# redmod-team/SympGPR

Measured on AMD Instinct MI355X. Metric: Gram-build GB/s + Cholesky fp64 TFLOP/s at N=65536 d=2; |alpha-alpha_ref|/|alpha_ref|, higher is better.
Workload: dtype f64

## Files before the change

### sympgpr_amd/csrc/chol.hip

```cpp
#include <algorithm>
#include <cstdlib>
#include <mutex>
#include <vector>

#include "cholq.h"
#include "common.h"
#include "gemm_tile.h"
#include "leaf.h"

namespace sgpr {

namespace {

using namespace leaf;


__global__ __launch_bounds__(LT) void leaf_kernel(int nb, double *A, size_t lda, double *inv,
                                                  int *dinfo, int goff, int mode,
                                                  unsigned long long *stamps)
{
    __shared__ double s[LEAF_LDS];
    if (nb == LEAF) leaf_body(s, (int)LEAF, A, lda, inv, dinfo, goff, mode, stamps);
    else            leaf_body(s, nb, A, lda, inv, dinfo, goff, mode, stamps);
}
// ... 476 lines not shown
            idx[0] = F0 + cp * PW_MAX + g;
            return panel_wait_ge(a.flags, idx, 1, 3, a.dinfo, sh + 1, a.abort);
        };
        for (int c = 0; c + 1 < g; ++c) {
            double *X = tileptr(g, c);
            XTile x;
            CTile cd;
            if (!wait_helper(c)) return false;
            asm volatile("s_waitcnt vmcnt(0)" ::: "memory");
            __syncthreads();
            trsm_prefetch(X, a.lda, x);
            diag_prefetch(tileptr(g, g), a.lda, cd);
            idx[0] = E0 + c;
            if (!panel_wait(a.flags, idx, 1, a.dinfo, sh + 1, a.abort)) return false;
            trsm_solve(s, tileptr(c, c), a.inv + (size_t)c * LEAF * LEAF, a.lda, x);
            trsm_store(X, a.lda, x);
            panel_publish_wt(a.flags + F0 + g * PW_MAX + c);
            diag_update_global(s, x, cd, tileptr(g, g), a.lda);
            if (c == 0 && a.NH > 0) claim_tiles();
            int cnt = 0;
            for (int cc = c + 1; cc < g; ++cc)
                if (!((helped >> cc) & 1u)) idx[cnt++] = F0 + cc * PW_MAX + c;
            if (cnt && !panel_wait(a.flags, idx, cnt, a.dinfo, sh + 1, a.abort)) return false;
            for (int t = 1; t < g - c; ++t)
                if (!((helped >> (c + t)) & 1u))
                    panel_product(s, -1.0, X, a.lda, tileptr(c + t, c), a.lda, 1.0, tileptr(g, c + t), a.lda);
        }
        if (g > 0) {
            const int c = g - 1;
            double *X = tileptr(g, c);
            XTile x;
            CTile cd;
            if (!wait_helper(c)) return false;
            asm volatile("s_waitcnt vmcnt(0)" ::: "memory");
            __syncthreads();
            trsm_prefetch(X, a.lda, x);
            diag_prefetch(tileptr(g, g), a.lda, cd);
            idx[0] = E0 + c;
            if (dbg) a.dbg[16 * g + 2] = __builtin_amdgcn_s_memrealtime();
            if (!panel_wait(a.flags, idx, 1, a.dinfo, sh + 1, a.abort)) return false;
            if (dbg) a.dbg[16 * g + 0] = __builtin_amdgcn_s_memrealtime();
            trsm_solve(s, tileptr(c, c), a.inv + (size_t)c * LEAF * LEAF, a.lda, x, a.dbg ? a.dbg + 16 * g + 6 : nullptr);
            trsm_store(X, a.lda, x);
            if (dbg) a.dbg[16 * g + 1] = __builtin_amdgcn_s_memrealtime();
            diag_update_into_leaf(s, x, cd, a.dbg ? a.dbg + 16 * g + 8 : nullptr);
            if (tid == 0) __hip_atomic_store((gint *)(a.flags + F0 + g * PW_MAX + c), 1, __ATOMIC_RELAXED, __HIP_MEMORY_SCOPE_AGENT);
        }
        asm volatile("s_waitcnt vmcnt(0)" ::: "memory");
        __syncthreads();
        if (dbg) a.dbg[16 * g + 4] = __builtin_amdgcn_s_memrealtime();
        leaf_body(s, (int)LEAF, tileptr(g, g), a.lda,
                  a.inv + (size_t)g * LEAF * LEAF, a.dinfo, a.goff + g * LEAF, (int)LEAF_FACTOR, nullptr,
                  a.flags + E0 + g, g > 0, dbg ? a.dbg + 16 * g + 11 : nullptr);
        panel_publish(a.flags + 2 + g);
        if (a.abort && tid == 0)
            __hip_atomic_fetch_add((gint *)(a.abort + (cholq::Q_PROG - cholq::Q_ABORT)), 1, __ATOMIC_RELAXED, __HIP_MEMORY_SCOPE_AGENT);
        if (dbg) a.dbg[16 * g + 5] = __builtin_amdgcn_s_memrealtime();
        if (cen && tid == 0) cen[2] = __builtin_amdgcn_s_memrealtime();
        return true;
    }
    if (g < W + a.NH) {
        int h = g - W, cp = 1, gg = 2;
        while (h >= W - 1 - cp) { h -= W - 1 - cp; ++cp; }
        gg = cp + 1 + h;
        int *word = a.flags + F0 + cp * PW_MAX + gg;
        if (tid == 0) sh[1] = atomicCAS(word, 0, 1);
        __syncthreads();
        const int old = sh[1];
        __syncthreads();
        if (old != 0) return true;
        if (a.ver) {
            idx[0] = ((a.ver_i0 + (gg >> 1)) * a.ver_ld + a.ver_j0 + cp) * (int)cholq::VS;
            if (!panel_wait_ge(a.ver, idx, 1, a.ver_need, a.dinfo, sh + 1, a.abort)) return false;
        }
        for (int c = 0; c < cp; ++c) {
            idx[0] = F0 + gg * PW_MAX + c;
            idx[1] = F0 + cp * PW_MAX + c;
            if (!panel_wait(a.flags, idx, 2, a.dinfo, sh + 1, a.abort)) return false;
            panel_product(s, -1.0, tileptr(gg, c), a.lda, tileptr(cp, c), a.lda, 1.0, tileptr(gg, cp), a.lda);
        }
        panel_publish_val(word, 3);
        return true;
    }
    const int gb = g - a.NH;
    if (a.tiles) {
        const int nbel = R - W, ntiles = nbel * W;
        int *const counter = a.flags + 2 * PFLAG_STRIDE - 1;
        for (;;) {
            if (tid == 0) sh[1] = atomicAdd(counter, 1);
            __syncthreads();
            const int q = sh[1];
            __syncthreads();
            if (q >= ntiles) return true;
            const int cp = q / nbel, r = W + q % nbel;
            const int pword = PFLAG_STRIDE + (r - W);
            if (a.ver) {
                idx[0] = ((a.ver_i0 + (r >> 1)) * a.ver_ld + a.ver_j0 + cp) * (int)cholq::VS;
                if (!panel_wait_ge(a.ver, idx, 1, a.ver_need, a.dinfo, sh + 1, a.abort)) return false;
            }
            for (int c = 0; c < cp; ++c) {
                idx[0] = pword;
                if (!panel_wait_ge(a.flags, idx, 1, c + 1, a.dinfo, sh + 1, a.abort)) return false;
                idx[0] = F0 + cp * PW_MAX + c;
                if (!panel_wait(a.flags, idx, 1, a.dinfo, sh + 1, a.abort)) return false;
                panel_product(s, -1.0, tileptr(r, c), a.lda, tileptr(cp, c), a.lda, 1.0, tileptr(r, cp), a.lda);
            }
            {
                double *X = tileptr(r, cp);
                XTile x;
                asm volatile("s_waitcnt vmcnt(0)" ::: "memory");
                __syncthreads();
                trsm_prefetch(X, a.lda, x);
                idx[0] = E0 + cp;
                if (!panel_wait(a.flags, idx, 1, a.dinfo, sh + 1, a.abort)) return false;
                trsm_solve(s, tileptr(cp, cp), a.inv + (size_t)cp * LEAF * LEAF, a.lda, x);
                trsm_store(X, a.lda, x);
            }
            asm volatile("s_waitcnt vmcnt(0)" ::: "memory");
            __syncthreads();
            if (tid == 0) __hip_atomic_store((gint *)(a.flags + pword), cp + 1, __ATOMIC_RELAXED, __HIP_MEMORY_SCOPE_AGENT);
            if (cp == W - 1) {
                if (a.tver) panel_publish_val(a.tver + (size_t)(a.tver_r0 + r) * cholq::VS, a.tver_val);
                if (a.abort && tid == 0)
                    __hip_atomic_fetch_add((gint *)(a.abort + (cholq::Q_PROG - cholq::Q_ABORT)), 1, __ATOMIC_RELAXED, __HIP_MEMORY_SCOPE_AGENT);
            }
        }
    }
    const int nw = G - W;
    const int r_first = W + (gb - W), r_step = nw > 0 ? nw : R;
    if (a.ver) {
        const int vi = a.ver_i0 + (r_first >> 1);
        for (int c = 0; c < W; ++c) idx[c] = (vi * a.ver_ld + a.ver_j0 + c) * (int)cholq::VS;
        if (r_first < R && !panel_wait_ge(a.ver, idx, W, a.ver_need, a.dinfo, sh + 1, a.abort)) return false;
    }
    const bool below_early = a.below_early != 0;
    for (int c = 0; c < W; ++c) {
        bool have_inv = false, have_early = false, have_rows = false;
        for (int r = r_first; r < R; r += r_step) {
            double *X = tileptr(r, c);
            if (c == W - 1 || below_early) {
                XTile x;
                asm volatile("s_waitcnt vmcnt(0)" ::: "memory");
                __syncthreads();
                trsm_prefetch(X, a.lda, x);
                if (!have_early) {
                    idx[0] = E0 + c;
                    if (!panel_wait(a.flags, idx, 1, a.dinfo, sh + 1, a.abort)) return false;
                    have_early = true;
                }
                trsm_solve(s, tileptr(c, c), a.inv + (size_t)c * LEAF * LEAF, a.lda, x);
                trsm_store(X, a.lda, x);
                if (c == W - 1) continue;
            } else {
                if (!have_inv) {
                    idx[0] = 2 + c;
                    if (!panel_wait(a.flags, idx, 1, a.dinfo, sh + 1, a.abort)) return false;
                    have_inv = true;
                }
                panel_product(s, 1.0, X, a.lda, a.inv + (size_t)c * LEAF * LEAF, (size_t)LEAF, 0.0, X, a.lda);
            }
            for (int t = 1; t <= W - 1 - c; ++t) {
                if (t == 1 && !have_rows) {
                    int cnt = 0;
                    for (int cc = c + 1; cc < W; ++cc) idx[cnt++] = F0 + cc * PW_MAX + c;
                    if (cnt && !panel_wait(a.flags, idx, cnt, a.dinfo, sh + 1, a.abort)) return false;
                    have_rows = true;
                }
                panel_product(s, -1.0, X, a.lda, tileptr(c + t, c), a.lda, 1.0, tileptr(r, c + t), a.lda);
            }
        }
    }
    if (a.tver && r_first < R) panel_publish_val(a.tver + (size_t)(a.tver_r0 + r_first) * cholq::VS, a.tver_val);
    if (a.abort && tid == 0)
        __hip_atomic_fetch_add((gint *)(a.abort + (cholq::Q_PROG - cholq::Q_ABORT)), 1, __ATOMIC_RELAXED, __HIP_MEMORY_SCOPE_AGENT);
    if (cen && tid == 0) cen[2] = __builtin_amdgcn_s_memrealtime();
    return true;
}

__global__ __launch_bounds__(LT) void panel_kernel(const PanelArgs a)
{
    __shared__ double s[LEAF * ILD];
    __shared__ int sh[2];
    static_assert(2 * tile::BK * 2 * (LEAF + tile::PAD) <= LEAF_LDS && LEAF_LDS <= LEAF * ILD, "product staging and the leaf fit the buffer");
    const int tid = threadIdx.x;
    const int W = a.W, G = a.G;
    if (tid == 0) {
        int t = -1;
        if ((blockIdx.x & 7) == 0) {
            t = atomicAdd(a.flags, 1);
            if (t >= W) t = -1;
        }
        if (t < 0) t = W + atomicAdd(a.flags + 1, 1);
        sh[0] = t;
    }
    __syncthreads();
    const int g = sh[0];
    __syncthreads();
    if (g >= G + a.NH) return;
    (void)panel_strip(a, g, s, sh);
}

struct PanelSeq {
    double *A;
    size_t lda;
    int nblk;
    int nblk_all;
    const int *pstart;
    double *inv;
    int *dinfo;
    int goff;
    int *flags;
    const int *ver;
    int ver_ld;
    int *tver;
    int *abort;
    unsigned long long *census;
    int helpers, tiles;
};

__global__ __launch_bounds__(LT) void panel_seq_kernel(const PanelSeq q)
{
    __shared__ double s[LEAF * ILD];
    __shared__ int sh[2];
    const int g = blockIdx.x;
    for (int k = 0; k < q.nblk; ++k) {
        const int k0 = q.pstart[k], w = q.pstart[k + 1] - k0, wnext = k + 1 < q.nblk_all ? q.pstart[k + 2] - q.pstart[k + 1] : 0;
        PanelArgs a{};
        a.P = q.A + k0 + (size_t)k0 * q.lda; a.lda = q.lda;
        a.W = w / LEAF;
        a.R = a.G = (w + wnext) / LEAF;
        a.below_early = q.tiles;
        a.NH = (q.helpers && a.W > 2 && a.G + (a.W - 1) * (a.W - 2) / 2 <= (int)gridDim.x) ? (a.W - 1) * (a.W - 2) / 2 : 0;
        if (q.tiles && wnext > 0 && a.W >= 2 && (int)gridDim.x - a.W - a.NH >= 1) {
            a.tiles = 1;
            a.G = a.W + min((int)gridDim.x - a.W - a.NH, (a.R - a.W) * a.W);
        }
        a.inv = q.inv + (size_t)(k0 / LEAF) * LEAF * LEAF;
        a.dinfo = q.dinfo; a.goff = q.goff + k0;
        a.flags = q.flags + (size_t)(k0 / LEAF) * PFLAG_STRIDE;
        a.dbg = nullptr;
        a.ver = q.ver; a.ver_ld = q.ver_ld; a.ver_i0 = k0 / cholq::TM; a.ver_j0 = k0 / cholq::TN; a.ver_need = k0 / LEAF;
        a.tver = q.tver; a.tver_r0 = k0 / LEAF; a.tver_val = (k0 + w) / LEAF;
        a.abort = q.abort;
        a.census = (q.census && k < (int)cholq::TRACE_PANELS) ? q.census + 4 * cholq::TRACE_PANEL_WGS * (size_t)k : nullptr;
        if (g < a.G + a.NH && !panel_strip(a, g, s, sh)) return;
        asm volatile("s_waitcnt vmcnt(0)" ::: "memory");
        __syncthreads();
    }
}

struct PanelBatch {
    double *A;
    size_t stride_a, lda;
    double *inv;
    size_t stride_inv;
    int *flags;
    int *info;
    int *ticket;
    int W, nbatch;
    int R;
    int k0;
    int G;
};

__global__ __launch_bounds__(LT) void panel_batch_kernel(const PanelBatch q)
{
    __shared__ double s[LEAF * ILD];
    __shared__ int sh[2];
    if (threadIdx.x == 0) sh[0] = atomicAdd(q.ticket, 1);
    __syncthreads();
    const int t = sh[0];
    __syncthreads();
    const int p = t / q.G, g = t - p * q.G;
    if (p >= q.nbatch) return;
    PanelArgs a{};
    a.P = q.A + (size_t)p * q.stride_a + (size_t)q.k0 + (size_t)q.k0 * q.lda; a.lda = q.lda;
    a.W = q.W; a.R = q.R; a.G = q.G;
    a.inv = q.inv + (size_t)p * q.stride_inv + (size_t)(q.k0 / (int)LEAF) * LEAF * LEAF;
    a.dinfo = q.info + p; a.goff = q.k0;
    a.flags = q.flags + (size_t)p * PFLAG_STRIDE;
    a.below_early = 1;
    (void)panel_strip(a, g, s, sh);
}

inline int split(int n)
{
    int n1 = ((n / 2 + LEAF - 1) / LEAF) * LEAF;
    if (n1 >= n) n1 -= LEAF;
    return n1;
}

struct Ctx {
    double *inv;
    int *dinfo;
    hipStream_t st;
    int la_max = 0;
    int *flags = nullptr;
    void *qws = nullptr;
};

int potrf_lookahead(int n, double *A, size_t lda, const Ctx &c, int nb, int off0);
inline int la_block(int n) { return n <= 4096 ? 256 : (n <= 24576 ? 512 : (n <= 40960 ? 1024 : 2048)); }

int trsm_rec(int m, int n, const double *L, size_t ldl, double *B, size_t ldb, int off, const Ctx &c)
{
    if (n <= LEAF) {
        return gemm_nt(m, n, n, 1.0, B, ldb, c.inv + (size_t)(off / LEAF) * LEAF * LEAF, LEAF, 0.0,
                       B, ldb, 0, 0, c.st);
    }
    const int n1 = split(n), n2 = n - n1;
    int rc = trsm_rec(m, n1, L, ldl, B, ldb, off, c);
    if (rc) return rc;
    rc = gemm_nt(m, n2, n1, -1.0, B, ldb, L + n1, ldl, 1.0, B + (size_t)n1 * ldb, ldb, 0, 0, c.st);
    if (rc) return rc;
    return trsm_rec(m, n2, L + n1 + (size_t)n1 * ldl, ldl, B + (size_t)n1 * ldb, ldb, off + n1, c);
}

int trsm_rl_rec(int m, int n, const double *L, size_t ldl, double *B, size_t ldb, int off, const Ctx &c)
{
    if (n <= LEAF)
        return gemm_nn(m, n, n, 1.0, B, ldb, c.inv + (size_t)(off / LEAF) * LEAF * LEAF, LEAF, 0.0, B, ldb, c.st);
    const int n1 = split(n), n2 = n - n1;
    int rc = trsm_rl_rec(m, n2, L + n1 + (size_t)n1 * ldl, ldl, B + (size_t)n1 * ldb, ldb, off + n1, c);
    if (rc) return rc;
    rc = gemm_nn(m, n1, n2, -1.0, B + (size_t)n1 * ldb, ldb, L + n1, ldl, 1.0, B, ldb, c.st);
    if (rc) return rc;
    return trsm_rl_rec(m, n1, L, ldl, B, ldb, off, c);
}

int potrf_rec(int n, double *A, size_t lda, int off, const Ctx &c)
{
    if (n <= LEAF) {
        hipLaunchKernelGGL(leaf_kernel, dim3(1), dim3(LT), 0, c.st, n, A, lda,
                           c.inv + (size_t)(off / LEAF) * LEAF * LEAF, c.dinfo, off, (int)LEAF_FACTOR,
                           (unsigned long long *)nullptr);
        SGPR_CHECK_LAUNCH();
        return 0;
    }
    if (n > 4 * LEAF && n <= c.la_max) return potrf_lookahead(n, A, lda, c, 0, off);
    const int n1 = split(n), n2 = n - n1;
    double *A21 = A + n1, *A22 = A + n1 + (size_t)n1 * lda;
    int rc = potrf_rec(n1, A, lda, off, c);
    if (rc) return rc;
    rc = trsm_rec(n2, n1, A, lda, A21, lda, off, c);
    if (rc) return rc;
    rc = gemm_nt(n2, n2, n1, -1.0, A21, lda, A21, lda, 1.0, A22, lda, 1, 0, c.st);
    if (rc) return rc;
    return potrf_rec(n2, A22, lda, off + n1, c);
}

int trsv_n_rec(int n, const double *L, size_t ldl, double *b, int off, const Ctx &c)
{
    if (n <= LEAF) {
        hipLaunchKernelGGL(leaf_matvec_kernel, dim3(1), dim3(MV_T), 0, c.st, n,
                           c.inv + (size_t)(off / LEAF) * LEAF * LEAF, b, 0);
        SGPR_CHECK_LAUNCH();
        return 0;
    }
    if (n <= TRSV_BLOCK) {
        hipLaunchKernelGGL(trsv_block_kernel, dim3(1), dim3(MV_T), 0, c.st, n, L, ldl,
                           c.inv + (size_t)(off / LEAF) * LEAF * LEAF, b, 0);
        SGPR_CHECK_LAUNCH();
        return 0;
    }
    const int n1 = split(n), n2 = n - n1;
    int rc = trsv_n_rec(n1, L, ldl, b, off, c);
    if (rc) return rc;
    rc = gemv_n_sub(n2, n1, L + n1, ldl, b, b + n1, c.st);
    if (rc) return rc;
    return trsv_n_rec(n2, L + n1 + (size_t)n1 * ldl, ldl, b + n1, off + n1, c);
}

int trsv_t_rec(int n, const double *L, size_t ldl, double *b, int off, const Ctx &c)
{
    if (n <= LEAF) {
        hipLaunchKernelGGL(leaf_matvec_kernel, dim3(1), dim3(MV_T), 0, c.st, n,
                           c.inv + (size_t)(off / LEAF) * LEAF * LEAF, b, 1);
        SGPR_CHECK_LAUNCH();
        return 0;
    }
    if (n <= TRSV_BLOCK) {
        hipLaunchKernelGGL(trsv_block_kernel, dim3(1), dim3(MV_T), 0, c.st, n, L, ldl,
                           c.inv + (size_t)(off / LEAF) * LEAF * LEAF, b, 1);
        SGPR_CHECK_LAUNCH();
        return 0;
    }
    const int n1 = split(n), n2 = n - n1;
    int rc = trsv_t_rec(n2, L + n1 + (size_t)n1 * ldl, ldl, b + n1, off + n1, c);
    if (rc) return rc;
    rc = gemv_t_sub(n2, n1, L + n1, ldl, b + n1, b, c.st);
    if (rc) return rc;
    return trsv_t_rec(n1, L, ldl, b, off, c);
}

int leaves_invert_only(int n, double *L, size_t ldl, const Ctx &c)
{
    for (int off = 0; off < n; off += LEAF) {
        const int nb = n - off < LEAF ? n - off : LEAF;
        hipLaunchKernelGGL(leaf_kernel, dim3(1), dim3(LT), 0, c.st, nb, L + off + (size_t)off * ldl, ldl,
                           c.inv + (size_t)(off / LEAF) * LEAF * LEAF, c.dinfo, off,
                           (int)LEAF_INVERT_ONLY, (unsigned long long *)nullptr);
        SGPR_CHECK_LAUNCH();
    }
    return 0;
}

inline size_t inv_bytes(int n)
{
    return (size_t)((n + LEAF - 1) / LEAF) * LEAF * LEAF * sizeof(double);
}
inline size_t flag_bytes(int n)
{
    return (((size_t)((n + LEAF - 1) / LEAF) * PFLAG_STRIDE * sizeof(int)) + 255) / 256 * 256;
}


}

inline size_t pub_bytes(int n) { return ((size_t)2 * n * sizeof(double) + 255) / 256 * 256; }
size_t potrf_workspace(int n) { return n <= 0 ? 256 : inv_bytes(n) + flag_bytes(n) + pub_bytes(n) + cholq::ws_bytes(n) + 256; }

namespace {

struct EventPool {
    std::vector<hipEvent_t> ev;
    size_t top = 0;
};
thread_local EventPool t_event_pool[64];

struct EventSet {
    std::vector<hipEvent_t> ev;
    EventPool *pool = nullptr;
    size_t base = 0;
    int create(size_t count)
    {
        int dev = 0;
        SGPR_HIP(hipGetDevice(&dev));
        if (dev < 0 || dev >= 64) { set_error("potrf: device index out of range"); return SGPR_E_ARG; }
        pool = &t_event_pool[dev];
        base = pool->top;
        while (pool->ev.size() < base + count) {
            hipEvent_t e = nullptr;
            SGPR_HIP(hipEventCreateWithFlags(&e, hipEventDisableTiming));
            pool->ev.push_back(e);
        }
        pool->top = base + count;
        ev.assign(pool->ev.begin() + (long)base, pool->ev.begin() + (long)(base + count));
        return 0;
    }
    ~EventSet()
    {
        if (pool) pool->top = base;
    }
};
struct StreamJoin {
    hipStream_t side, caller;
    hipEvent_t ev;
    ~StreamJoin()
    {
        if (hipEventRecord(ev, side) != hipSuccess || hipStreamWaitEvent(caller, ev, 0) != hipSuccess)
            (void)hipStreamSynchronize(side);
        gemm_set_overlap(0);
    }
};

hipStream_t g_side[64] = {};
std::mutex g_side_mu;

void release_all_streams_at_exit();
void register_exit_release()
{
    static std::once_flag once;
    std::call_once(once, [] { (void)atexit(release_all_streams_at_exit); });
}

int side_stream(hipStream_t caller, hipStream_t *out, int *dev_out)
{
    hipStream_t *const side = g_side;
    int dev = -1;
    if (caller) {
        SGPR_HIP(hipStreamGetDevice(caller, &dev));
    } else {
        SGPR_HIP(hipGetDevice(&dev));
    }
    if (dev < 0 || dev >= 64) { set_error("potrf: device index out of range"); return SGPR_E_ARG; }
    std::lock_guard<std::mutex> lock(g_side_mu);
    if (!side[dev]) {
        int cur = -1, lo = 0, hi = 0;
        SGPR_HIP(hipGetDevice(&cur));
        if (cur != dev) SGPR_HIP(hipSetDevice(dev));
        hipError_t e = hipDeviceGetStreamPriorityRange(&lo, &hi);
        if (e == hipSuccess) e = hipStreamCreateWithPriority(&side[dev], hipStreamNonBlocking, hi);
        if (e == hipSuccess) register_exit_release();
        if (cur != dev) (void)hipSetDevice(cur);
        SGPR_HIP(e);
    }
    *out = side[dev];
    *dev_out = dev;
    return 0;
}

struct QueueDevice {
    std::mutex mu;
    hipEvent_t done = nullptr;
    int ncu = 0;
    hipStream_t workers[4] = {}, panels[4] = {};
    bool overlap_ok[4] = {};
    bool failed = false;
};
QueueDevice g_qdev[64];

__global__ void overlap_probe_kernel(int *w, int me)
{
    __hip_atomic_store((gint *)(w + me), 1, __ATOMIC_RELAXED, __HIP_MEMORY_SCOPE_AGENT);
    const unsigned long long t0 = __builtin_amdgcn_s_memrealtime();
    int seen = 0;
    while (!(seen = __hip_atomic_load((gint *)(w + 1 - me), __ATOMIC_RELAXED, __HIP_MEMORY_SCOPE_AGENT))) {
        __builtin_amdgcn_s_sleep(32);
        if (__builtin_amdgcn_s_memrealtime() - t0 > 5000000ull) break;
    }
    w[2 + me] = seen ? 1 : 2;
}
static bool queue_overlap_ok(hipStream_t sw, hipStream_t sp)
{
    int *w = nullptr;
    if (hipMalloc((void **)&w, 4 * sizeof(int)) != hipSuccess) { (void)hipGetLastError(); return false; }
    int h[4] = {0, 0, 0, 0};
    bool ok = hipMemset(w, 0, sizeof(h)) == hipSuccess;
    if (ok) {
        hipLaunchKernelGGL(overlap_probe_kernel, dim3(1), dim3(1), 0, sp, w, 0);
        hipLaunchKernelGGL(overlap_probe_kernel, dim3(1), dim3(1), 0, sw, w, 1);
        ok = hipGetLastError() == hipSuccess && hipStreamSynchronize(sp) == hipSuccess && hipStreamSynchronize(sw) == hipSuccess &&
             hipMemcpy(h, w, sizeof(h), hipMemcpyDeviceToHost) == hipSuccess && h[2] == 1 && h[3] == 1;
    }
    (void)hipFree(w);
    (void)hipGetLastError();
    return ok;
}

int queue_streams(QueueDevice &qd, int dev, int R, hipStream_t *sw, hipStream_t *sp)
{
    if (!qd.workers[R - 1]) {
        int cur = -1;
        SGPR_HIP(hipGetDevice(&cur));
        if (cur != dev) SGPR_HIP(hipSetDevice(dev));
        const int words = qd.ncu / 32;
        std::vector<uint32_t> mp((size_t)words, 0u), mw((size_t)words, 0xFFFFFFFFu);
        for (int b = 0; b < 8 * R; ++b) { mp[b / 32] |= 1u << (b % 32); mw[b / 32] &= ~(1u << (b % 32)); }
        hipError_t e = hipExtStreamCreateWithCUMask(&qd.panels[R - 1], (uint32_t)words, mp.data());
        if (e == hipSuccess) e = hipExtStreamCreateWithCUMask(&qd.workers[R - 1], (uint32_t)words, mw.data());
        if (e == hipSuccess) register_exit_release();
        if (cur != dev) (void)hipSetDevice(cur);
        if (e != hipSuccess) {
            (void)hipGetLastError();
            qd.failed = true;
            return SGPR_E_HIP;
        }
    }
    if (!qd.overlap_ok[R - 1]) {
        if (!queue_overlap_ok(qd.workers[R - 1], qd.panels[R - 1])) {
            qd.failed = true;
            return SGPR_E_HIP;
        }
        qd.overlap_ok[R - 1] = true;
    }
    *sw = qd.workers[R - 1];
    *sp = qd.panels[R - 1];
    return 0;
}

thread_local bool t_last_potrf_used_queue = false;

int potrf_queue(int n, double *A, size_t lda, const Ctx &c, int off0)
{
    int dev = -1;
    if (c.st) {
        SGPR_HIP(hipStreamGetDevice(c.st, &dev));
    } else {
        SGPR_HIP(hipGetDevice(&dev));
    }
    if (dev < 0 || dev >= 64) { set_error("potrf: device index out of range"); return SGPR_E_ARG; }
    QueueDevice &qd = g_qdev[dev];
    std::lock_guard<std::mutex> lock(qd.mu);
    if (qd.failed) return 1;
    if (!qd.ncu) {
        SGPR_HIP(hipDeviceGetAttribute(&qd.ncu, hipDeviceAttributeMultiprocessorCount, dev));
        SGPR_HIP(hipEventCreateWithFlags(&qd.done, hipEventDisableTiming));
        SGPR_HIP(hipEventRecord(qd.done, c.st));
    }
    if (qd.ncu % 64 != 0 || qd.ncu < 64) { qd.failed = true; return 1; }
    const std::vector<int> starts = cholq::default_starts(n);
    int band = 0;
    for (size_t k = 0; k + 1 < starts.size(); ++k)
        band = std::max(band, (starts[k + 1] - starts[k] + (k + 2 < starts.size() ? starts[k + 2] - starts[k + 1] : 0)) / LEAF);
    static const int q_helpers = (int)tune("q_helpers", 0), q_tiles = (int)tune("q_tiles", 0);
    int nh_max = 0;
    for (size_t k = 0; k + 1 < starts.size(); ++k) {
        const int W = (starts[k + 1] - starts[k]) / LEAF;
        if (q_helpers && W > 2) nh_max = std::max(nh_max, (W - 1) * (W - 2) / 2);
    }
    const int pgrid = band + nh_max + std::max(0, q_tiles);
    const int R = (pgrid + 7) / 8;
    if (R > 4) return 1;
    hipStream_t sw = nullptr, sp = nullptr;
    if (queue_streams(qd, dev, R, &sw, &sp)) return 1;
    static const int qslack = (int)tune("q_slack", 0);
    const int nworkers = qd.ncu - 8 * R - std::max(0, std::min(qslack, 64));
    const cholq::Plan *plan = cholq::get_plan(n, nworkers);
// ... 537 lines not shown
```

Measured before the change: 71.59.

## Fuse recursive panel TRSM into a single strip-parallel kernel

Adds a kernel in which each workgroup owns one LEAF-row strip of B and walks all LEAF column blocks itself. For each block it applies the GEMM update from the earlier solved blocks, then multiplies by the precomputed inverse diagonal block. This replaces the recursive trsm_rec chain of many small gemm launches with one launch, cutting launch overhead and serialization. In exchange the in-strip work runs sequentially and parallelism is limited to m/LEAF workgroups. It relies on in-workgroup fences for ordering and is gated by alignment and size checks.

```diff
diff --git a/sympgpr_amd/csrc/chol.hip b/sympgpr_amd/csrc/chol.hip
--- a/sympgpr_amd/csrc/chol.hip
+++ b/sympgpr_amd/csrc/chol.hip
@@ -802,8 +802,64 @@
 int potrf_lookahead(int n, double *A, size_t lda, const Ctx &c, int nb, int off0);
 inline int la_block(int n) { return n <= 4096 ? 256 : (n <= 24576 ? 512 : (n <= 40960 ? 1024 : 2048)); }
 
+struct TrsmBelowArgs {
+    int m, n;
+    const double *L;
+    size_t ldl;
+    const double *inv;
+    double *B;
+    size_t ldb;
+};
+
+__global__ __launch_bounds__(256, 2) void trsm_below_kernel(const TrsmBelowArgs a)
+{
+    __shared__ double smem[2 * tile::BK * 2 * (LEAF + tile::PAD)];
+    const int strip = blockIdx.x;
+    const bool full = (strip + 1) * (int)LEAF <= a.m;
+    tile::GemmArgs g{};
+    g.m = a.m; g.n = LEAF;
+    g.lda = a.ldb; g.ldc = a.ldb;
+    auto product = [&]() {
+        if (full) tile::gemm_body_dma<LEAF, LEAF, 2>(g, smem, strip, 0);
+        else      tile::gemm_body<LEAF, LEAF, false>(g, smem, strip, 0);
+        asm volatile("s_waitcnt vmcnt(0)" ::: "memory");
+        __syncthreads();
+        if (threadIdx.x == 0) {
+            __builtin_amdgcn_fence(__ATOMIC_ACQUIRE, "agent");
+            asm volatile("s_waitcnt vmcnt(0)" ::: "memory");
+        }
+        __syncthreads();
+    };
+    const int nc = a.n / (int)LEAF;
+    for (int s = 1; s < 2 * nc; ++s) {
+        const int c = s >> 1;
+        double *Bc = a.B + (size_t)c * LEAF * a.ldb;
+        g.C = Bc;
+        if (s & 1) {
+            g.k = LEAF; g.alpha = 1.0; g.beta = 0.0;
+            g.A = Bc; g.B = a.inv + (size_t)c * LEAF * LEAF; g.ldb = LEAF;
+        } else {
+            g.k = c * (int)LEAF; g.alpha = -1.0; g.beta = 1.0;
+            g.A = a.B; g.B = a.L + (size_t)c * LEAF; g.ldb = a.ldl;
+        }
+        product();
+    }
+}
+
+inline bool trsm_below_ok(int m, int n, const double *L, size_t ldl, const double *B, size_t ldb, int off)
+{
+    return m > 0 && n > (int)LEAF && n <= PW_MAX * (int)LEAF && n % LEAF == 0 && off % LEAF == 0 &&
+           ((ldl | ldb) & 1) == 0 && ((((uintptr_t)L | (uintptr_t)B) & 15) == 0);
+}
+
 int trsm_rec(int m, int n, const double *L, size_t ldl, double *B, size_t ldb, int off, const Ctx &c)
 {
+    if (trsm_below_ok(m, n, L, ldl, B, ldb, off) && tune("trsm_below", 1) != 0) {
+        const TrsmBelowArgs ta{m, n, L, ldl, c.inv + (size_t)(off / LEAF) * LEAF * LEAF, B, ldb};
+        hipLaunchKernelGGL(trsm_below_kernel, dim3((m + (int)LEAF - 1) / (int)LEAF), dim3(256), 0, c.st, ta);
+        SGPR_CHECK_LAUNCH();
+        return 0;
+    }
     if (n <= LEAF) {
         return gemm_nt(m, n, n, 1.0, B, ldb, c.inv + (size_t)(off / LEAF) * LEAF * LEAF, LEAF, 0.0,
                        B, ldb, 0, 0, c.st);
```

Result: no change. 71.81 (median of 6 runs) (+0.3%).
